# sampotter/butterfly

Measured on AMD Instinct MI355X. Metric: butterfly matvecs/sec (2D Helmholtz HODBF apply), higher is better.
Workload: dtype c128

## Files before the change

butterfly_amd/csrc/bfhip_device.hip:

```cpp

#include <hip/hip_runtime.h>
#include <type_traits>
#include <vector>
#include <stdint.h>
#include <stdio.h>
#include <stdlib.h>

#include "bfhip_internal.h"
#include "bfhip_stage_c128.h"
#include "../../include/bfhip_abi.h"
#include "bfhip_hip.h"
#include "../../include/bfhip_synth.h"

#define BF_WAVES_PER_WG 4
#define BF_WAVE_LDS_BYTES (BF_XCAP * 16)

struct __attribute__((aligned(8))) bfC64 { float re, im; };
struct bfC64Acc { double re, im; };
__device__ __forceinline__ bfC64Acc &operator+=(bfC64Acc &a, bfC64Acc b) { a.re += b.re; a.im += b.im; return a; }

template <int DT> struct Traits;
template <> struct Traits<BFHIP_C128> { using S = double; using A = double; static constexpr int EPL = 1; static constexpr bool CPLX = true; };
template <> struct Traits<BFHIP_F64> { using S = double; using A = double; using E = double; using EA = double; static constexpr int EPL = 2; static constexpr bool CPLX = false; };
template <> struct Traits<BFHIP_F32> { using S = float; using A = float; using E = float; using EA = float; static constexpr int EPL = 4; static constexpr bool CPLX = false; };
template <> struct Traits<BFHIP_C64> { using S = float; using A = double; using E = bfC64; using EA = bfC64Acc; static constexpr int EPL = 2; static constexpr bool CPLX = true; };

__device__ __forceinline__ double bfMac(double acc, double a, double x) { return fma(a, x, acc); }
__device__ __forceinline__ float bfMac(float acc, float a, float x) { return fma(a, x, acc); }
__device__ __forceinline__ bfC64Acc bfMac(bfC64Acc acc, bfC64 a, bfC64 x) {
  double const ar = a.re, ai = a.im, xr = x.re, xi = x.im;
  acc.re = fma(ar, xr, acc.re); acc.re = fma(-ai, xi, acc.re);
  acc.im = fma(ar, xi, acc.im); acc.im = fma(ai, xr, acc.im);
  return acc;
}
__device__ __forceinline__ double bfToAcc(double v) { return v; }
__device__ __forceinline__ float bfToAcc(float v) { return v; }
__device__ __forceinline__ bfC64Acc bfToAcc(bfC64 v) { return bfC64Acc{v.re, v.im}; }
__device__ __forceinline__ double bfFromAcc(double v) { return v; }
__device__ __forceinline__ float bfFromAcc(float v) { return v; }
__device__ __forceinline__ bfC64 bfFromAcc(bfC64Acc v) { return bfC64{(float)v.re, (float)v.im}; }
__device__ __forceinline__ double bfShflXor(double v, int m, int w) { return __shfl_xor(v, m, w); }
__device__ __forceinline__ float bfShflXor(float v, int m, int w) { return __shfl_xor(v, m, w); }
__device__ __forceinline__ bfC64Acc bfShflXor(bfC64Acc v, int m, int w) { return bfC64Acc{__shfl_xor(v.re, m, w), __shfl_xor(v.im, m, w)}; }

template <int NC, typename A, typename S>
__device__ __forceinline__ void bfMacN(A *acc, S const *a, S const *x) {
  if constexpr (NC == 1) {
    acc[0] = fma((A)a[0], (A)x[0], acc[0]);
  } else {
    A const ar = a[0], ai = a[1], xr = x[0], xi = x[1];
    acc[0] = fma(ar, xr, acc[0]); acc[0] = fma(-ai, xi, acc[0]);
    acc[1] = fma(ar, xi, acc[1]); acc[1] = fma(ai, xr, acc[1]);
  }
}

template <typename V> __device__ __forceinline__ V bfLoadStreamV(V const *p) {
  static_assert(sizeof(V) == 16, "one 16-byte lane load");
#if BF_STREAM_NT
  bf_u4 raw = __builtin_nontemporal_load((bf_u4 const *)p);
  V v;
  __builtin_memcpy(&v, &raw, 16);
  return v;
#else
  return *p;
#endif
}

template <bool TL>
__device__ __forceinline__ void bfStageBodyC128(StageParams const &p, double2 (*lds)[BF_XCAP], uint64_t *timeline) {
  int const wave = threadIdx.x >> 6;
  int const lane = threadIdx.x & 63;
  uint32_t const item = __builtin_amdgcn_readfirstlane(blockIdx.x * BF_C128_WG_WAVES + wave);
  if (item >= p.numItems) return;
  BfDevItem const it = p.items[item];
  bfItemC128<TL, false>(p, it, item, lds[wave], lane, timeline, BfNoHook());
}

#ifdef BF_C128_WAVES
#define BF_C128_ATTR __attribute__((amdgpu_waves_per_eu(BF_C128_WAVES, BF_C128_WAVES)))
#else
#define BF_C128_ATTR
#endif
__global__ __launch_bounds__(BF_C128_WG_WAVES * 64) BF_C128_ATTR void bfStageKernelC128(StageParams p) {
  __shared__ __attribute__((aligned(16))) double2 lds[BF_C128_WG_WAVES][BF_XCAP];
  bfStageBodyC128<false>(p, lds, nullptr);
}

#include "bfhip_stage_mfma.h"
#include "bfhip_stage_mfma_blocks.h"

template <int DT, int MR>
__device__ __forceinline__ void bfRowMajorPiece(void const *rowpV, uint32_t upr, typename Traits<DT>::E const *xin, uint32_t n,
                                                uint32_t nrhs, int lane, typename Traits<DT>::EA *racc) {
  using E = typename Traits<DT>::E;
  constexpr int EPL = Traits<DT>::EPL;
  struct __attribute__((aligned(16))) V { E v[EPL]; };
  struct __attribute__((packed, aligned(sizeof(E)))) VU { E v[EPL]; };
  char const *rowp = (char const *)rowpV;
  constexpr int UNR = MR <= 2 ? 4 : 2;
  uint32_t const rowBytes = upr * 16u;
  uint32_t const full = nrhs == 1 ? n / EPL : 0;
  uint32_t u = (uint32_t)lane;
  if (UNR > 1) {
#pragma unroll 1
    for (; u + 64u * (UNR - 1) < full; u += 64u * UNR) {
      V a[UNR][MR];
      VU xv[UNR];
#pragma unroll
      for (int k = 0; k < UNR; ++k) {
#pragma unroll
        for (int r = 0; r < MR; ++r) a[k][r] = bfLoadStreamV((V const *)(rowp + ((uint32_t)r * rowBytes + (u + 64u * k) * 16u)));
      }
#pragma unroll
      for (int k = 0; k < UNR; ++k) xv[k] = *(VU const *)((char const *)xin + (u + 64u * k) * 16u);
#pragma unroll
      for (int k = 0; k < UNR; ++k) {
#pragma unroll
        for (int r = 0; r < MR; ++r) {
#pragma unroll
          for (int e = 0; e < EPL; ++e) racc[r] = bfMac(racc[r], a[k][r].v[e], xv[k].v[e]);
        }
      }
    }
  }
#pragma unroll 1
  for (; u < full; u += 64u) {
    V a[MR];
#pragma unroll
    for (int r = 0; r < MR; ++r) a[r] = bfLoadStreamV((V const *)(rowp + ((uint32_t)r * rowBytes + u * 16u)));
    VU const xv = *(VU const *)((char const *)xin + u * 16u);
#pragma unroll
    for (int r = 0; r < MR; ++r) {
#pragma unroll
      for (int e = 0; e < EPL; ++e) racc[r] = bfMac(racc[r], a[r].v[e], xv.v[e]);
    }
  }
#pragma unroll 1
  for (; u < upr; u += 64u) {
    V a[MR];
#pragma unroll
    for (int r = 0; r < MR; ++r) a[r] = bfLoadStreamV((V const *)(rowp + ((uint32_t)r * rowBytes + u * 16u)));
    E xv[EPL];
#pragma unroll
    for (int e = 0; e < EPL; ++e) xv[e] = u * EPL + e < n ? xin[(uint64_t)(u * EPL + e) * nrhs] : E{};
#pragma unroll
    for (int r = 0; r < MR; ++r) {
#pragma unroll
      for (int e = 0; e < EPL; ++e) racc[r] = bfMac(racc[r], a[r].v[e], xv[e]);
    }
  }
}

template <int DT>
__device__ __forceinline__ void bfStageBodySmall(StageParams const &p, uint32_t const bid) {
  using E = typename Traits<DT>::E;
  using EA = typename Traits<DT>::EA;
  constexpr int EPL = Traits<DT>::EPL;
  constexpr int RMAX = 2 * EPL;
  struct __attribute__((aligned(16))) V { E v[EPL]; };
  int const wave = threadIdx.x >> 6;
  int const lane = threadIdx.x & 63;
  uint32_t const item0 = __builtin_amdgcn_readfirstlane((bid * BF_WAVES_PER_WG + wave) * 4u);
  if (item0 >= p.numItems) return;
  uint32_t const gid = (uint32_t)lane >> 4, gl = (uint32_t)lane & 15u;
  uint32_t const idx = item0 + gid;
  bool const valid = idx < p.numItems;
  BfDevItem it = p.items[valid ? idx : p.numItems - 1];
  uint32_t const mr = valid ? (it.mrFlags & 0xffffu) : 0u;
  uint32_t const np = valid ? it.numPieces : 0u;
  BfDevPiece my;
  my.dataOff = 0; my.inOff = 0; my.ncols = 0; my.flags = 0; my.ld = 0;
  if (gl < np) my = p.pieces[it.pieceBegin + gl];
  uint32_t npMax = 0;
#pragma unroll
  for (int k = 0; k < 4; ++k) {
    uint32_t const v = (uint32_t)__builtin_amdgcn_readlane((int)np, 16 * k);
    npMax = v > npMax ? v : npMax;
  }
  V const *arena = (V const *)p.arena;
  uint32_t const nrhs = p.nrhs;
  E *out = (it.mrFlags & BF_ITEM_OUT_Y) ? (E *)p.y : (E *)p.temp;
  for (uint32_t q = 0; q < nrhs; ++q) {
    EA racc[RMAX];
#pragma unroll
    for (int r = 0; r < RMAX; ++r) racc[r] = EA{};
    EA ident{};
    for (uint32_t k = 0; k < npMax; ++k) {
      int const from = (int)(gid * 16u + k);
      uint32_t const flags = (uint32_t)__shfl((int)my.flags, from, 64);
      uint32_t const inOff = (uint32_t)__shfl((int)my.inOff, from, 64);
      uint32_t const ncols = (uint32_t)__shfl((int)my.ncols, from, 64);
      uint32_t const ld = (uint32_t)__shfl((int)my.ld, from, 64);
      uint32_t const dLo = (uint32_t)__shfl((int)(uint32_t)my.dataOff, from, 64);
      uint32_t const dHi = (uint32_t)__shfl((int)(uint32_t)(my.dataOff >> 32), from, 64);
      if (k >= np) continue;
      E const *xin = ((flags & BF_PIECE_IN_X) ? (E const *)p.x : (E const *)p.temp) + ((uint64_t)inOff * nrhs + q);
      if (flags & BF_PIECE_IDENTITY) {
        if (gl < mr) ident += bfToAcc(xin[(uint64_t)gl * nrhs]);
        continue;
      }
      uint32_t const upr = ld / EPL;
      V const *base = arena + (((uint64_t)dHi << 32) | dLo) / EPL;
#pragma unroll 1
      for (uint32_t u = gl; u < upr; u += 16u) {
        V a[RMAX];
#pragma unroll
        for (int r = 0; r < RMAX; ++r) if ((uint32_t)r < mr) a[r] = bfLoadStreamV(base + (uint64_t)r * upr + u);
        E xv[EPL];
#pragma unroll
        for (int e = 0; e < EPL; ++e) xv[e] = u * EPL + e < ncols ? xin[(uint64_t)(u * EPL + e) * nrhs] : E{};
#pragma unroll
        for (int r = 0; r < RMAX; ++r)
          if ((uint32_t)r < mr) {
#pragma unroll
            for (int e = 0; e < EPL; ++e) racc[r] = bfMac(racc[r], a[r].v[e], xv[e]);
          }
      }
    }
    EA mine = ident;
// ... 128 lines not shown
          if (base && (pc.dataOff != nextOff || base + pc.ncols > BF_MERGE_COLS)) break;
          if (base == 0) data0 = pc.dataOff;
          nextOff = pc.dataOff + (uint64_t)mrPad * pc.ncols;
#pragma unroll
          for (int t = 0; t < XS; ++t) {
            uint32_t const J = (uint32_t)lane + 64u * t - base;
            if (J < pc.ncols) { src[t] = pc.inOff + J; srcX = (pc.flags & BF_PIECE_IN_X) ? srcX | (1u << t) : srcX & ~(1u << t); }
          }
          base += pc.ncols;
        }
        uint32_t n;
        V const *ap = arena + data0 / EPL + lc;
        if (wideCols) {
          E const *xin = (wideFlags & BF_PIECE_IN_X) ? (E const *)p.x : (E const *)p.temp;
          xin += (uint64_t)wideIn * nrhs + q;
          n = wideCols;
          waveSync();
          for (uint32_t j = lane; j < n; j += 64) xs[j] = xin[(uint64_t)j * nrhs];
          waveSync();
        } else if (base) {
          n = base;
          bool const tiny = n <= 2 * g;
          V a2[2];
          if (tiny) {
#pragma unroll
            for (int kk = 0; kk < 2; ++kk) {
#pragma unroll
              for (int e = 0; e < EPL; ++e) a2[kk].v[e] = E{};
              if (active && c + kk * g < n) a2[kk] = bfLoadStreamV(ap + (uint64_t)kk * G);
            }
          }
          E xg[XS];
#pragma unroll
          for (int t = 0; t < XS; ++t)
            xg[t] = src[t] != ~0u ? (((srcX >> t) & 1u) ? (E const *)p.x : (E const *)p.temp)[(uint64_t)src[t] * nrhs + q] : E{};
          waveSync();
#pragma unroll
          for (int t = 0; t < XS; ++t) if ((uint32_t)lane + 64u * t < n) xs[lane + 64 * t] = xg[t];
          waveSync();
          if (tiny) {
#pragma unroll
            for (int kk = 0; kk < 2; ++kk) {
              E xv = (active && c + kk * g < n) ? xs[c + kk * g] : E{};
#pragma unroll
              for (int e = 0; e < EPL; ++e) acc[e] = bfMac(acc[e], a2[kk].v[e], xv);
            }
            continue;
          }
        } else {
          continue;
        }
        uint32_t const nfull = n / g;
        uint32_t j = c;
        uint32_t s = 0;
        V a8[BF_REAL_UNROLL];
#pragma unroll 1
        for (; s + BF_REAL_UNROLL <= nfull; s += BF_REAL_UNROLL) {
#pragma unroll
          for (int k = 0; k < BF_REAL_UNROLL; ++k) a8[k] = bfLoadStreamV(ap + (uint64_t)(s + k) * G);
#pragma unroll
          for (int k = 0; k < BF_REAL_UNROLL; ++k) {
            E const xv = xs[j];
#pragma unroll
            for (int e = 0; e < EPL; ++e) acc[e] = bfMac(acc[e], a8[k].v[e], xv);
            j += g;
          }
        }
        if (s < nfull) {
          uint32_t const left = nfull - s;
#pragma unroll
          for (int k = 0; k < BF_REAL_UNROLL - 1; ++k)
            if ((uint32_t)k < left) a8[k] = bfLoadStreamV(ap + (uint64_t)(s + k) * G);
#pragma unroll
          for (int k = 0; k < BF_REAL_UNROLL - 1; ++k)
            if ((uint32_t)k < left) {
              E const xv = xs[j];
#pragma unroll
              for (int e = 0; e < EPL; ++e) acc[e] = bfMac(acc[e], a8[k].v[e], xv);
              j += g;
            }
        }
        uint32_t const rem = n - nfull * g;
        if (active && c < rem) {
          V a = bfLoadStreamV(ap + (uint64_t)nfull * G);
          E xv = xs[j];
#pragma unroll
          for (int e = 0; e < EPL; ++e) acc[e] = bfMac(acc[e], a.v[e], xv);
        }
      }
    }
    waveSync();
#pragma unroll
    for (int e = 0; e < EPL; ++e) xa[lane * EPL + e] = acc[e];
    waveSync();
    for (uint32_t row = lane; row < mr; row += 64) {
      EA sum{};
      for (uint32_t cc = 0; cc < g; ++cc) sum += xa[cc * mrPad + row];
      out[((uint64_t)it.outOff + row) * nrhs + q] = bfFromAcc(sum);
    }
  }
}

template <int DT>
__global__ __launch_bounds__(BF_WAVES_PER_WG * 64) void bfStageKernelReal(StageParams p) {
  __shared__ __attribute__((aligned(16))) unsigned char ldsRaw[BF_WAVES_PER_WG][BF_WAVE_LDS_BYTES];
  bfStageBodyReal<DT>(p, blockIdx.x, ldsRaw);
}

template <int DT>
__global__ __launch_bounds__(BF_WAVES_PER_WG * 64) __attribute__((amdgpu_waves_per_eu(4, 8))) void bfStageKernelRealBoth(StageParams pr, StageParams ps, uint32_t gridReal) {
  __shared__ __attribute__((aligned(16))) unsigned char ldsRaw[BF_WAVES_PER_WG][BF_WAVE_LDS_BYTES];
  if (blockIdx.x < gridReal) bfStageBodyReal<DT>(pr, blockIdx.x, ldsRaw);
  else bfStageBodySmall<DT>(ps, blockIdx.x - gridReal);
}


#define BF_T_COLS 16
#ifndef BF_T_WIDE_NT
#define BF_T_WIDE_NT 0
#endif
#ifndef BF_T_WIDE_R
#define BF_T_WIDE_R 4
#endif

template <int DT, int R, int NQ, bool COOP, bool ONE, typename CoopBuf>
__device__ __forceinline__ void bfStageBodyT(StageParams const &p, uint32_t const bid, CoopBuf &coopBuf) {
  constexpr int C = 64 / R;
  using S = typename Traits<DT>::S;
  using A = typename Traits<DT>::A;
  constexpr int EPL = Traits<DT>::EPL;
  constexpr int NC = Traits<DT>::CPLX ? 2 : 1;
  constexpr int UNIT = EPL * NC;
  struct __attribute__((aligned(16))) U { S v[UNIT]; };
  int const wave = threadIdx.x >> 6;
  int const lane = threadIdx.x & 63;
  bool const coop = COOP && bid < p.coopItems;
  uint32_t item = __builtin_amdgcn_readfirstlane(coop ? bid : p.coopItems + (bid - p.coopItems) * BF_WAVES_PER_WG + wave);
  if (item >= p.numItems) return;
  uint32_t const wsel = coop ? (uint32_t)wave : 0u, wmask = coop ? BF_WAVES_PER_WG - 1u : 0u;
  BfDevItem const it = p.items[item];
  uint32_t const mr = it.mrFlags & 0xffffu;
  uint32_t const c4 = lane / R, r = lane % R;
  uint32_t jcol[NQ];
#pragma unroll
  for (int cq = 0; cq < NQ; ++cq) jcol[cq] = c4 + C * cq < mr ? c4 + C * cq : mr - 1;
  U const *arena = (U const *)p.arena;
  uint32_t const nrhs = ONE ? 1u : p.nrhs;
  S *out = (it.mrFlags & BF_ITEM_OUT_Y) ? (S *)p.y : (S *)p.temp;
  uint32_t const nq = (mr + C - 1) / C;

  constexpr int CG_RM = (NQ * C) / EPL > 64 ? 64 : (NQ * C) / EPL;
  constexpr int RL_RM = 64 / CG_RM;
  uint32_t const cgRm = lane % CG_RM, rlRm = lane / CG_RM;

  for (uint32_t q = 0; q < nrhs; ++q) {
    A acc[NQ][NC];
#pragma unroll
    for (int cq = 0; cq < NQ; ++cq)
#pragma unroll
      for (int k = 0; k < NC; ++k) acc[cq][k] = 0;
    A racc[EPL][NC];
#pragma unroll
    for (int e = 0; e < EPL; ++e)
#pragma unroll
      for (int k = 0; k < NC; ++k) racc[e][k] = 0;
    bool anyRowMajor = false;
    for (uint32_t wbase = 0; wbase < it.numPieces; wbase += 64) {
      uint32_t const wn = it.numPieces - wbase < 64 ? it.numPieces - wbase : 64;
      BfPieceWin const win = bfPieceWinLoad(p.pieces + it.pieceBegin + wbase, wn, lane);
      uint32_t const pstep = wmask + 1u;
      for (uint32_t pi = wsel; pi < wn; pi += pstep) {
        BfDevPiece const pc = bfPieceWinGet(win, pi);
        S const *xin = (pc.flags & BF_PIECE_IN_X) ? (S const *)p.x : (S const *)p.temp;
        xin += ((uint64_t)pc.inOff * nrhs + q) * NC;
        if (pc.flags & BF_PIECE_IDENTITY) {
          if (r == 0) {
#pragma unroll
            for (int cq = 0; cq < NQ; ++cq)
#pragma unroll
              for (int k = 0; k < NC; ++k) acc[cq][k] += (A)xin[(uint64_t)jcol[cq] * nrhs * NC + k];
          }
          continue;
        }
        if constexpr (EPL > 1) {
          if (pc.flags & BF_PIECE_ROWMAJOR) {
            anyRowMajor = true;
            uint32_t const n = pc.ncols;
            uint32_t const cgc = cgRm < (mr + EPL - 1) / EPL ? cgRm : (mr - 1) / EPL;
            U const *src = arena + pc.dataOff / EPL + cgc;
            uint32_t const rowUnits = pc.ld / EPL;
            constexpr int ITERS = (2 * EPL + RL_RM - 1) / RL_RM;
            bool dual = pi + pstep < wn;
            BfDevPiece pc2 = pc;
            if (dual) {
              pc2 = bfPieceWinGet(win, pi + pstep);
              dual = (pc2.flags & (BF_PIECE_ROWMAJOR | BF_PIECE_IDENTITY)) == BF_PIECE_ROWMAJOR;
            }
            U a[ITERS], a2[ITERS];
            S xv[ITERS][NC], xv2[ITERS][NC];
#pragma unroll
            for (int i = 0; i < ITERS; ++i) {
              uint32_t const srow = rlRm + (uint32_t)i * RL_RM, sc = srow < n ? srow : n - 1;
              a[i] = bfLoadStreamV(src + (uint64_t)sc * rowUnits);
#pragma unroll
              for (int k = 0; k < NC; ++k) {
                S const xr = xin[(uint64_t)sc * nrhs * NC + k];
                xv[i][k] = srow < n ? xr : (S)0;
              }
            }
            if (dual) {
              S const *xin2 = ((pc2.flags & BF_PIECE_IN_X) ? (S const *)p.x : (S const *)p.temp) + ((uint64_t)pc2.inOff * nrhs + q) * NC;
              uint32_t const n2 = pc2.ncols;
              U const *src2 = arena + pc2.dataOff / EPL + cgc;
              uint32_t const rowUnits2 = pc2.ld / EPL;
#pragma unroll
              for (int i = 0; i < ITERS; ++i) {
                uint32_t const srow = rlRm + (uint32_t)i * RL_RM, sc = srow < n2 ? srow : n2 - 1;
                a2[i] = bfLoadStreamV(src2 + (uint64_t)sc * rowUnits2);
#pragma unroll
                for (int k = 0; k < NC; ++k) {
                  S const xr = xin2[(uint64_t)sc * nrhs * NC + k];
                  xv2[i][k] = srow < n2 ? xr : (S)0;
                }
              }
            }
#pragma unroll
            for (int i = 0; i < ITERS; ++i)
#pragma unroll
              for (int e = 0; e < EPL; ++e) bfMacN<NC>(racc[e], &a[i].v[e * NC], xv[i]);
            if (dual) {
#pragma unroll
              for (int i = 0; i < ITERS; ++i)
#pragma unroll
                for (int e = 0; e < EPL; ++e) bfMacN<NC>(racc[e], &a2[i].v[e * NC], xv2[i]);
              pi += pstep;
            }
            continue;
          }
        }
        uint32_t const stride = pc.ld / EPL;
        uint32_t const n = pc.ncols;
        uint32_t const units = (n + EPL - 1) / EPL;
        U const *src = arena + pc.dataOff / EPL;
        for (uint32_t rb = 0; rb < units; rb += R) {
          uint32_t const ru = rb + r < units ? rb + r : units - 1;
          U a[NQ];
#pragma unroll
          for (int cq = 0; cq < NQ; ++cq) if ((uint32_t)cq < nq) a[cq] = (R >= 16 || BF_T_WIDE_NT) ? bfLoadStreamV(src + jcol[cq] * stride + ru) : src[jcol[cq] * stride + ru];
          S xv[UNIT];
#pragma unroll
          for (int e = 0; e < EPL; ++e) {
            uint32_t const row = (rb + r) * EPL + e;
            uint32_t const rowc = row < n ? row : n - 1;
#pragma unroll
            for (int k = 0; k < NC; ++k) {
              S const v = xin[(uint64_t)rowc * nrhs * NC + k];
              xv[e * NC + k] = row < n ? v : (S)0;
            }
          }
#pragma unroll
          for (int cq = 0; cq < NQ; ++cq) {
            if ((uint32_t)cq >= nq) continue;
#pragma unroll
            for (int e = 0; e < EPL; ++e) bfMacN<NC>(acc[cq], &a[cq].v[e * NC], &xv[e * NC]);
          }
        }
      }
    }
#pragma unroll
    for (int m = 1; m < R; m <<= 1)
#pragma unroll
      for (int cq = 0; cq < NQ; ++cq)
#pragma unroll
        for (int k = 0; k < NC; ++k) acc[cq][k] += __shfl_xor(acc[cq][k], m, R);
    if constexpr (EPL > 1) {
      if (anyRowMajor) {
#pragma unroll
        for (int e = 0; e < EPL; ++e)
#pragma unroll
          for (int k = 0; k < NC; ++k)
#pragma unroll
            for (int m = CG_RM; m < 64; m <<= 1) racc[e][k] += __shfl_xor(racc[e][k], m, 64);
#pragma unroll
        for (int cq = 0; cq < NQ; ++cq) {
          uint32_t const col = c4 + C * cq < mr ? c4 + C * cq : 0;
#pragma unroll
          for (int e = 0; e < EPL; ++e)
#pragma unroll
            for (int k = 0; k < NC; ++k) {
              A const t = __shfl(racc[e][k], (int)(col / EPL), 64);
              if ((int)(col % EPL) == e) acc[cq][k] += t;
            }
        }
      }
    }
    if (COOP && coop) {
      if (r == 0) {
#pragma unroll
        for (int cq = 0; cq < NQ; ++cq)
#pragma unroll
          for (int k = 0; k < NC; ++k) coopBuf[wave][c4 + C * cq][k] = acc[cq][k];
      }
      __syncthreads();
      if (wave == 0 && r == 0) {
#pragma unroll
        for (int cq = 0; cq < NQ; ++cq)
#pragma unroll
          for (int k = 0; k < NC; ++k) {
            A t = coopBuf[0][c4 + C * cq][k];
#pragma unroll
            for (int w = 1; w < BF_WAVES_PER_WG; ++w) t += coopBuf[w][c4 + C * cq][k];
            acc[cq][k] = t;
          }
      }
      __syncthreads();
      if (wave != 0) continue;
    }
    if (r == 0) {
#pragma unroll
      for (int cq = 0; cq < NQ; ++cq)
        if (c4 + C * cq < mr)
#pragma unroll
          for (int k = 0; k < NC; ++k) out[(((uint64_t)it.outOff + c4 + C * cq) * nrhs + q) * NC + k] = (S)acc[cq][k];
    }
  }
}

template <int DT, int R, int NQ, bool COOP, bool ONE>
__global__ __launch_bounds__(BF_WAVES_PER_WG * 64) void bfStageKernelT(StageParams p) {
  using A = typename Traits<DT>::A;
  constexpr int NC = Traits<DT>::CPLX ? 2 : 1;
  __shared__ A coopBuf[COOP ? BF_WAVES_PER_WG : 1][COOP ? NQ * (64 / R) : 1][NC];
  bfStageBodyT<DT, R, NQ, COOP, ONE>(p, blockIdx.x, coopBuf);
}

template <int DT, bool ONE>
__global__ __launch_bounds__(BF_WAVES_PER_WG * 64) void bfStageKernelTBoth(StageParams pn, StageParams pw, uint32_t gridNarrow) {
  using A = typename Traits<DT>::A;
  constexpr int NC = Traits<DT>::CPLX ? 2 : 1;
  __shared__ A coopBuf[BF_WAVES_PER_WG][64][NC];
  if (blockIdx.x < gridNarrow) bfStageBodyT<DT, 16, 4, true, ONE>(pn, blockIdx.x, coopBuf);
  else bfStageBodyT<DT, BF_T_WIDE_R, BF_T_WIDE_R, true, ONE>(pw, blockIdx.x - gridNarrow, coopBuf);
}

struct ReduceBatch {
  uint32_t count, nrhs;
  void const *temp;
  struct Entry {
    uint32_t const *rowInterval, *ivBegin;
    int64_t const *srcBias;
    uint64_t numRows;
    void *dest;
    uint32_t blockBegin, pad;
  } e[BF_REDUCE_BATCH];
};

template <typename T, int NC, bool LONG = false>
__global__ __launch_bounds__(256) void bfReduceKernel(ReduceBatch const B) {
  using TA = typename std::conditional<NC == 2 && sizeof(T) == 4, double, T>::type;
  uint32_t k = 0;
  while (k + 1 < B.count && B.e[k + 1].blockBegin <= blockIdx.x) ++k;
  ReduceBatch::Entry const &E = B.e[k];
  uint32_t const nrhs = B.nrhs;
  uint64_t idx = (uint64_t)(blockIdx.x - E.blockBegin) * 256 + threadIdx.x;
  uint64_t total = E.numRows * nrhs;
  if (idx >= total) return;
  uint64_t row = idx / nrhs;
  uint32_t q = (uint32_t)(idx - row * nrhs);
  uint32_t iv = E.rowInterval[row];
  if (iv == 0xffffffffu) return;
  uint32_t b = E.ivBegin[iv], e = E.ivBegin[iv + 1];
  T const *temp = (T const *)B.temp;
  T *dest = (T *)E.dest;
  TA acc[NC];
#pragma unroll
  for (int c = 0; c < NC; ++c) acc[c] = 0;
  uint32_t s = b;
  if (LONG) {
    for (; s + 32 <= e; s += 32) {
      T v[32][NC];
#pragma unroll
      for (int k = 0; k < 32; ++k) {
        T const *src = temp + ((uint64_t)(E.srcBias[s + k] + (int64_t)row) * nrhs + q) * NC;
#pragma unroll
        for (int c = 0; c < NC; ++c) v[k][c] = src[c];
      }
#pragma unroll
      for (int k = 0; k < 32; ++k)
#pragma unroll
        for (int c = 0; c < NC; ++c) acc[c] += v[k][c];
    }
  }
#pragma unroll 8
  for (; s < e; ++s) {
    T const *src = temp + ((uint64_t)(E.srcBias[s] + (int64_t)row) * nrhs + q) * NC;
#pragma unroll
    for (int c = 0; c < NC; ++c) acc[c] += src[c];
  }
#pragma unroll
  for (int c = 0; c < NC; ++c) dest[idx * NC + c] = (T)acc[c];
}

template <typename S>
__global__ __launch_bounds__(256) void bfScalePermuteKernel(S *dst, S const *src, S const *scale, int power, uint64_t const *perm, uint64_t n) {
  uint64_t const i = (uint64_t)blockIdx.x * 256 + threadIdx.x;
  if (i >= n) return;
  S v = src[i];
  if (scale) { S const g = scale[i]; v *= power == 2 ? g * g : g; }
  uint64_t const j = perm ? perm[i] : i;
  if (j < n) dst[j] = v;
}

template <int DT>
__global__ __launch_bounds__(256) void bfSynthKernel(void *arenaV, BfSynthPiece const *pieces, uint64_t seed) {
  using S = typename Traits<DT>::S;
  constexpr bool CPLX = Traits<DT>::CPLX;
  BfSynthPiece const pc = pieces[blockIdx.x];
  uint64_t total = pc.rowMajor ? (uint64_t)pc.mr * pc.ldr : (uint64_t)pc.mrPad * pc.ncols;
  S *dst = (S *)arenaV + pc.dataOff * (CPLX ? 2 : 1);
  for (uint64_t e = threadIdx.x; e < total; e += 256) {
    uint32_t col, r;
    if (pc.rowMajor) { r = (uint32_t)(e / pc.ldr); col = (uint32_t)(e - (uint64_t)r * pc.ldr); }
    else { col = (uint32_t)(e / pc.mrPad); r = (uint32_t)(e - (uint64_t)col * pc.mrPad); }
    S re = 0, im = 0;
    if (r < pc.mr && col < pc.ncols) {
      uint64_t idx = pc.vbase + (uint64_t)(pc.row0 + r) * pc.strideR + (uint64_t)(pc.col0 + col) * pc.strideC;
      re = (S)(bfhip_synth_value(seed, idx, 0) * pc.scale);
      if (CPLX) im = (S)(bfhip_synth_value(seed, idx, 1) * pc.scale);
    }
    if (CPLX) { dst[2 * e] = re; dst[2 * e + 1] = im; }
    else dst[e] = re;
  }
}


#define BF_REAL_CASES(DT, NAME) \
  case BFHIP_KERNEL_REAL_##NAME: hipLaunchKernelGGL(bfStageKernelReal<DT>, dim3(grid), dim3(BF_WAVES_PER_WG * 64), 0, s, p); break; \
  case BFHIP_KERNEL_SMALL_##NAME: hipLaunchKernelGGL(bfStageKernelSmall<DT>, dim3(grid), dim3(BF_WAVES_PER_WG * 64), 0, s, p); break; \
  case BFHIP_KERNEL_REALBOTH_##NAME: hipLaunchKernelGGL(bfStageKernelRealBoth<DT>, dim3(grid + grid2), dim3(BF_WAVES_PER_WG * 64), 0, s, p, p2, grid); break;
#define BF_T_CASES(DT, NAME) \
  case BFHIP_KERNEL_T_##NAME##_NARROW_N: hipLaunchKernelGGL((bfStageKernelT<DT, 16, 4, false, false>), dim3(grid), dim3(BF_WAVES_PER_WG * 64), 0, s, p); break; \
  case BFHIP_KERNEL_T_##NAME##_NARROW_ONE: hipLaunchKernelGGL((bfStageKernelT<DT, 16, 4, false, true>), dim3(grid), dim3(BF_WAVES_PER_WG * 64), 0, s, p); break; \
  case BFHIP_KERNEL_T_##NAME##_NARROW_COOP_N: hipLaunchKernelGGL((bfStageKernelT<DT, 16, 4, true, false>), dim3(grid), dim3(BF_WAVES_PER_WG * 64), 0, s, p); break; \
  case BFHIP_KERNEL_T_##NAME##_NARROW_COOP_ONE: hipLaunchKernelGGL((bfStageKernelT<DT, 16, 4, true, true>), dim3(grid), dim3(BF_WAVES_PER_WG * 64), 0, s, p); break; \
  case BFHIP_KERNEL_T_##NAME##_WIDE_N: hipLaunchKernelGGL((bfStageKernelT<DT, BF_T_WIDE_R, BF_T_WIDE_R, false, false>), dim3(grid), dim3(BF_WAVES_PER_WG * 64), 0, s, p); break; \
  case BFHIP_KERNEL_T_##NAME##_WIDE_ONE: hipLaunchKernelGGL((bfStageKernelT<DT, BF_T_WIDE_R, BF_T_WIDE_R, false, true>), dim3(grid), dim3(BF_WAVES_PER_WG * 64), 0, s, p); break; \
  case BFHIP_KERNEL_T_##NAME##_WIDE_COOP_N: hipLaunchKernelGGL((bfStageKernelT<DT, BF_T_WIDE_R, BF_T_WIDE_R, true, false>), dim3(grid), dim3(BF_WAVES_PER_WG * 64), 0, s, p); break; \
  case BFHIP_KERNEL_T_##NAME##_WIDE_COOP_ONE: hipLaunchKernelGGL((bfStageKernelT<DT, BF_T_WIDE_R, BF_T_WIDE_R, true, true>), dim3(grid), dim3(BF_WAVES_PER_WG * 64), 0, s, p); break;
#define BF_TBOTH_CASES(DT, NAME) \
  case BFHIP_KERNEL_TBOTH_##NAME##_N: hipLaunchKernelGGL((bfStageKernelTBoth<DT, false>), dim3(grid + grid2), dim3(BF_WAVES_PER_WG * 64), 0, s, p, p2, grid); break; \
  case BFHIP_KERNEL_TBOTH_##NAME##_ONE: hipLaunchKernelGGL((bfStageKernelTBoth<DT, true>), dim3(grid + grid2), dim3(BF_WAVES_PER_WG * 64), 0, s, p, p2, grid); break;
static int bfLaunchWaveStage(BfKernelLaunch const &L, BfLaunchArgs const *a, StageParams p, hipStream_t s) {
  bool const small = L.kernel >= BFHIP_KERNEL_SMALL_F64 && L.kernel <= BFHIP_KERNEL_SMALL_C64;
  uint32_t const perWg = small ? 4 * BF_WAVES_PER_WG : BF_WAVES_PER_WG;
  p.items = (BfDevItem const *)a->items + L.first[0];
  p.numItems = (uint32_t)L.count[0];
  p.coopItems = (uint32_t)L.coop[0];
  uint32_t const grid = (uint32_t)(L.coop[0] + (L.count[0] - L.coop[0] + perWg - 1) / perWg);
  StageParams p2 = p;
  uint32_t grid2 = 0;
  if (L.numRanges == 2) {
    bool const tboth = L.kernel >= BFHIP_KERNEL_TBOTH_F64_N && L.kernel <= BFHIP_KERNEL_TBOTH_C64_ONE;
    uint32_t const perWg2 = tboth ? BF_WAVES_PER_WG : 4 * BF_WAVES_PER_WG;
    p2.items = (BfDevItem const *)a->items + L.first[1];
    p2.numItems = (uint32_t)L.count[1];
    p2.coopItems = (uint32_t)L.coop[1];
    grid2 = (uint32_t)(L.coop[1] + (L.count[1] - L.coop[1] + perWg2 - 1) / perWg2);
  }
  switch (L.kernel) {
    BF_REAL_CASES(BFHIP_F64, F64) BF_REAL_CASES(BFHIP_F32, F32) BF_REAL_CASES(BFHIP_C64, C64)
    BF_T_CASES(BFHIP_C128, C128) BF_T_CASES(BFHIP_F64, F64) BF_T_CASES(BFHIP_F32, F32) BF_T_CASES(BFHIP_C64, C64)
    BF_TBOTH_CASES(BFHIP_F64, F64) BF_TBOTH_CASES(BFHIP_F32, F32) BF_TBOTH_CASES(BFHIP_C64, C64)
    default: return bfhipFail(BFABI_ERROR_RUNTIME_ERROR, "internal: kernel id %u is not a wavefront-per-item stage kernel", L.kernel);
  }
  return 0;
}
#undef BF_REAL_CASES
#undef BF_T_CASES
#undef BF_TBOTH_CASES

extern "C" {

// ... 180 lines not shown
```

butterfly_amd/csrc/bfhip_file.c:

```c
#include "bfhip_operator.h"
#include "../../include/bfhip_abi.h"

#include <stdio.h>
#include <stdlib.h>
#include <string.h>

#define BFHIP_FILE_MAGIC "BFHIPOP1"

typedef struct FileHeader {
  char magic[8];
  uint32_t version, dtype, srcDtype, elemSize, epl, xcap, hasTplan, reserved;
  uint64_t numRows, numCols, arenaElems, leafElems, numLeaves, leafBytesAlgorithmic;
} FileHeader;

typedef struct FilePlanHeader { uint64_t numStages, tempElems, numRows, numCols; uint32_t maxItemRows, transposed; } FilePlanHeader;
typedef struct FileStageHeader { uint64_t numItems, numPieces, leafElems, vecIn, vecOut, numReduce; uint32_t maxRows, reserved; } FileStageHeader;
typedef struct FileReduceHeader { uint64_t destOff, numRows, numIntervals, numSrc; uint32_t destSpace, reserved; } FileReduceHeader;

static int writeAll(FILE *fp, void const *p, size_t n) { return n == 0 || fwrite(p, 1, n, fp) == n ? 0 : bfhipFail(BFABI_ERROR_FILE_ERROR, "short write"); }
static int readAll(FILE *fp, void *p, size_t n) { return n == 0 || fread(p, 1, n, fp) == n ? 0 : bfhipFail(BFABI_ERROR_FILE_ERROR, "short read / truncated file"); }

static int writeDeviceArray(FILE *fp, void const *d, size_t bytes) {
  if (!bytes) return 0;
  size_t const chunk = (size_t)64 << 20;
  void *h = malloc(bytes < chunk ? bytes : chunk);
  if (!h) return bfhipFail(BFABI_ERROR_MEMORY_ERROR, "host OOM");
  int rc = 0;
  for (size_t off = 0; off < bytes && !rc; off += chunk) {
    size_t n = bytes - off < chunk ? bytes - off : chunk;
    rc = bfdevMemcpyD2H(h, (char const *)d + off, n);
    if (!rc) rc = writeAll(fp, h, n);
  }
  free(h);
  return rc;
}
static int readDeviceArray(FILE *fp, void **d, size_t bytes, uint64_t *meta) {
  int rc = bfdevMalloc(d, bytes + BF_ARENA_SLACK);
  if (rc || !bytes) return rc;
  if (meta) *meta += bytes;
  size_t const chunk = (size_t)64 << 20;
  void *h = malloc(bytes < chunk ? bytes : chunk);
  if (!h) return bfhipFail(BFABI_ERROR_MEMORY_ERROR, "host OOM");
  for (size_t off = 0; off < bytes && !rc; off += chunk) {
    size_t n = bytes - off < chunk ? bytes - off : chunk;
    rc = readAll(fp, h, n);
    if (!rc) rc = bfdevMemcpyH2D((char *)*d + off, h, n);
  }
  free(h);
  return rc;
}

static int savePlan(FILE *fp, BfPlan const *pl) {
  FilePlanHeader ph = {pl->numStages, pl->tempElems, pl->numRows, pl->numCols, pl->maxItemRows, (uint32_t)pl->transposed};
  int rc = writeAll(fp, &ph, sizeof ph);
  for (uint64_t s = 0; s < pl->numStages && !rc; ++s) {
    BfStage const *st = &pl->stages[s];
    FileStageHeader sh = {st->numItems, st->numPieces, st->leafElems, st->vecIn, st->vecOut, st->numReduce, st->maxRows, 0};
    rc = writeAll(fp, &sh, sizeof sh);
    if (!rc) rc = writeDeviceArray(fp, st->dItems, st->numItems * sizeof(BfDevItem));
    if (!rc) rc = writeDeviceArray(fp, st->dPieces, st->numPieces * sizeof(BfDevPiece));
    for (uint64_t r = 0; r < st->numReduce && !rc; ++r) {
      BfReduce const *rd = &st->reduce[r];
      FileReduceHeader rh = {rd->destOff, rd->numRows, rd->numIntervals, rd->numSrc, rd->destSpace, 0};
      rc = writeAll(fp, &rh, sizeof rh);
      if (!rc) rc = writeDeviceArray(fp, rd->dRowInterval, rd->numRows * 4);
      if (!rc) rc = writeDeviceArray(fp, rd->dIvBegin, (rd->numIntervals + 1) * 4);
      if (!rc) rc = writeDeviceArray(fp, rd->dSrcBias, rd->numSrc * 8);
    }
  }
  return rc;
}

static int readMetaArray(FILE *fp, void **d, void **h, size_t bytes, uint64_t *meta) {
  *h = NULL;
  int rc = bfdevMalloc(d, bytes);
  if (rc || !bytes) return rc;
  if (meta) *meta += bytes;
  *h = malloc(bytes);
  if (!*h) return bfhipFail(BFABI_ERROR_MEMORY_ERROR, "host OOM");
  if ((rc = readAll(fp, *h, bytes))) return rc;
  return bfdevMemcpyH2D(*d, *h, bytes);
}

static int fitsIn(uint64_t off, uint64_t ext, uint64_t len) { return off <= len && ext <= len - off; }
static uint64_t mulAddSat(uint64_t a, uint64_t b, uint64_t c) {
  uint64_t r;
  if (__builtin_mul_overflow(a, b, &r) || __builtin_add_overflow(r, c, &r)) return UINT64_MAX;
  return r;
}

static int validateStage(BfPlan const *pl, uint64_t arenaElems, BfStage const *st, BfDevItem const *items, BfDevPiece const *pieces) {
  uint64_t const inX = pl->numCols, outY = pl->numRows, temp = pl->tempElems;
  for (uint64_t i = 0; i < st->numItems; ++i) {
    BfDevItem const *it = &items[i];
    uint32_t const mr = it->mrFlags & 0xffffu;
    uint64_t const outLen = (it->mrFlags & BF_ITEM_OUT_Y) ? outY : temp;
    if (!mr || mr > pl->maxItemRows || mr > st->maxRows || (it->mrFlags & ~(0xffffu | BF_ITEM_OUT_Y | BF_ITEM_ROWMAJOR | BF_ITEM_MERGED | BF_ITEM_SMALL | BF_ITEM_TNARROW)) ||
        ((it->mrFlags & BF_ITEM_TNARROW) != 0) != (i < st->numNarrow) || ((it->mrFlags & BF_ITEM_TNARROW) && (!pl->transposed || mr > 16)) ||
        ((it->mrFlags & BF_ITEM_SMALL) != 0) != (i >= st->firstSmall) ||
        ((it->mrFlags & BF_ITEM_ROWMAJOR) && (pl->transposed || bfDtypeC128Layout(pl->dtype) || mr > 2 * pl->epl)) ||
        (pl->transposed && mr > 64) ||
        !fitsIn(it->outOff, mr, outLen) || !fitsIn(it->pieceBegin, it->numPieces, st->numPieces))
      return bfhipFail(BFABI_ERROR_FILE_ERROR, "corrupt operator file: item %llu out of bounds", (unsigned long long)i);
    uint32_t const mrPad = (mr + pl->epl - 1) / pl->epl * pl->epl;
    if (it->mrFlags & (BF_ITEM_MERGED | BF_ITEM_SMALL)) {
      int const sm = (it->mrFlags & BF_ITEM_SMALL) != 0;
      uint64_t next = 0, dense = 0;
      int const smRm = sm && (it->mrFlags & BF_ITEM_ROWMAJOR);
      int badm = pl->transposed || bfDtypeC128Layout(pl->dtype) || (!sm && (it->mrFlags & BF_ITEM_ROWMAJOR)) || it->numPieces > (sm ? BF_SMALL_PIECES : 64u) ||
                 (sm && (mr > 2 * pl->epl || !(it->mrFlags & BF_ITEM_ROWMAJOR)));
      for (uint32_t k = 0; k < it->numPieces && !badm; ++k) {
        BfDevPiece const *pc = &pieces[it->pieceBegin + k];
        if (pc->flags & BF_PIECE_IDENTITY) continue;
        if (!smRm && dense && pc->dataOff != next) badm = 1;
        next = mulAddSat(mrPad, pc->ncols, pc->dataOff); dense += pc->ncols;
      }
      if (badm || (!dense && !sm) || dense > (sm ? BF_SMALL_COLS : BF_MERGE_COLS))
        return bfhipFail(BFABI_ERROR_FILE_ERROR, "corrupt operator file: merged item %llu is not one block", (unsigned long long)i);
    }
    for (uint32_t k = 0; k < it->numPieces; ++k) {
      BfDevPiece const *pc = &pieces[it->pieceBegin + k];
      uint64_t const inLen = (pc->flags & BF_PIECE_IN_X) ? inX : temp;
      int bad = (pc->flags & ~(BF_PIECE_IN_X | BF_PIECE_IDENTITY | BF_PIECE_ROWMAJOR)) != 0;
      int const rm = (pc->flags & BF_PIECE_ROWMAJOR) != 0;
      if (!(pc->flags & BF_PIECE_IDENTITY) && !pl->transposed && rm != ((it->mrFlags & BF_ITEM_ROWMAJOR) != 0)) bad = 1;
      if (pc->flags & BF_PIECE_IDENTITY) bad |= !fitsIn(pc->inOff, mr, inLen);
      else if (pl->transposed && rm)
        bad |= !pc->ld || pc->ld % pl->epl || pc->dataOff % pl->epl || bfDtypeC128Layout(pl->dtype) || !pc->ncols ||
               !fitsIn(pc->dataOff, mulAddSat(pc->ncols - 1, pc->ld, (mr + pl->epl - 1) / pl->epl * pl->epl), arenaElems) ||
               !fitsIn(pc->inOff, pc->ncols, inLen);
      else if (rm)
        bad |= !pc->ncols || pc->ld % pl->epl || pc->ld < pc->ncols || pc->dataOff % pl->epl ||
               !fitsIn(pc->dataOff, mulAddSat(mr, pc->ld, 0), arenaElems) || !fitsIn(pc->inOff, pc->ncols, inLen);
      else if (pl->transposed)
        bad |= !pc->ld || pc->ld % pl->epl || pc->ncols > pc->ld || pc->dataOff % pl->epl ||
               !fitsIn(pc->dataOff, mulAddSat(mr - 1, pc->ld, (pc->ncols + pl->epl - 1) / pl->epl * pl->epl), arenaElems) ||
               !fitsIn(pc->inOff, pc->ncols, inLen);
      else
        bad |= !pc->ncols || pc->ncols > pl->xcap || pc->dataOff % pl->epl ||
               !fitsIn(pc->dataOff, mulAddSat(mrPad, pc->ncols, 0), arenaElems) || !fitsIn(pc->inOff, pc->ncols, inLen);
      if (bad) return bfhipFail(BFABI_ERROR_FILE_ERROR, "corrupt operator file: piece %u of item %llu out of bounds", k, (unsigned long long)i);
    }
  }
  return 0;
}

static int validateReduce(BfPlan const *pl, BfReduce const *rd, uint32_t const *rowInterval, uint32_t const *ivBegin, int64_t const *srcBias) {
  uint64_t const destLen = rd->destSpace == BF_SPACE_Y ? pl->numRows : pl->tempElems;
  if ((rd->destSpace != BF_SPACE_Y && rd->destSpace != BF_SPACE_TEMP) || !fitsIn(rd->destOff, rd->numRows, destLen) || rd->numIntervals > rd->numRows + 1)
    return bfhipFail(BFABI_ERROR_FILE_ERROR, "corrupt operator file: reduce destination out of bounds");
  if (ivBegin[0] != 0 || ivBegin[rd->numIntervals] > rd->numSrc) return bfhipFail(BFABI_ERROR_FILE_ERROR, "corrupt operator file: reduce interval table");
  for (uint64_t i = 0; i < rd->numIntervals; ++i)
    if (ivBegin[i + 1] < ivBegin[i]) return bfhipFail(BFABI_ERROR_FILE_ERROR, "corrupt operator file: reduce interval table not monotone");
  for (uint64_t r = 0; r < rd->numRows; ++r) {
    uint32_t const iv = rowInterval[r];
    if (iv == BF_REDUCE_SKIP) continue;
    if (iv >= rd->numIntervals) return bfhipFail(BFABI_ERROR_FILE_ERROR, "corrupt operator file: reduce row %llu", (unsigned long long)r);
    for (uint32_t k = ivBegin[iv]; k < ivBegin[iv + 1]; ++k) {
      int64_t src;
      if (__builtin_add_overflow(srcBias[k], (int64_t)r, &src) || src < 0 || (uint64_t)src >= pl->tempElems) return bfhipFail(BFABI_ERROR_FILE_ERROR, "corrupt operator file: reduce source out of bounds");
    }
  }
  return 0;
}

static int loadPlan(FILE *fp, BfhipOperator *op, BfPlan *pl, FileHeader const *fh, uint64_t arenaElems) {
  FilePlanHeader ph;
  int rc = readAll(fp, &ph, sizeof ph);
  if (rc) return rc;
  if (ph.numStages > (1u << 20) || ph.tempElems >= 0xffffffffu) return bfhipFail(BFABI_ERROR_FILE_ERROR, "corrupt plan header");
  pl->dtype = fh->dtype; pl->elemSize = fh->elemSize; pl->epl = fh->epl; pl->xcap = fh->xcap;
  pl->maxItemRows = ph.maxItemRows; pl->transposed = (int)ph.transposed;
  pl->numRows = ph.numRows; pl->numCols = ph.numCols; pl->numStages = ph.numStages; pl->tempElems = ph.tempElems;
  pl->arenaElems = pl->transposed ? 0 : arenaElems;
  pl->leafElems = fh->leafElems; pl->numLeaves = fh->numLeaves;
  if (pl->epl != 16 / pl->elemSize || pl->xcap != 256 || pl->maxItemRows > 64 * pl->epl || (pl->transposed && pl->maxItemRows > 128))
    return bfhipFail(BFABI_ERROR_FILE_ERROR, "corrupt plan header (lane granule / piece width / item height)");
  pl->stages = calloc(ph.numStages ? ph.numStages : 1, sizeof(BfStage));
  if (!pl->stages) return bfhipFail(BFABI_ERROR_MEMORY_ERROR, "host OOM");
  for (uint64_t s = 0; s < pl->numStages && !rc; ++s) {
    BfStage *st = &pl->stages[s];
    FileStageHeader sh;
    if ((rc = readAll(fp, &sh, sizeof sh))) break;
    if (sh.numItems > 0xffffffffu || sh.numPieces > 0xffffffffu || sh.numReduce > (1u << 20)) { rc = bfhipFail(BFABI_ERROR_FILE_ERROR, "corrupt stage header"); break; }
    st->numItems = sh.numItems; st->numPieces = sh.numPieces; st->leafElems = sh.leafElems; st->vecIn = sh.vecIn; st->vecOut = sh.vecOut;
    st->maxRows = sh.maxRows;
    void *hItems = NULL, *hPieces = NULL;
    rc = readMetaArray(fp, &st->dItems, &hItems, st->numItems * sizeof(BfDevItem), &op->metaBytes);
    if (!rc) rc = readMetaArray(fp, &st->dPieces, &hPieces, st->numPieces * sizeof(BfDevPiece), &op->metaBytes);
    if (!rc) {
      st->firstSmall = st->numItems;
      while (st->firstSmall && (((BfDevItem const *)hItems)[st->firstSmall - 1].mrFlags & BF_ITEM_SMALL)) --st->firstSmall;
      st->numNarrow = 0;
      while (st->numNarrow < st->numItems && (((BfDevItem const *)hItems)[st->numNarrow].mrFlags & BF_ITEM_TNARROW)) ++st->numNarrow;
      rc = validateStage(pl, arenaElems, st, hItems, hPieces);
      if (!rc && pl->transposed) {
        st->maxRowsRest = 0;
        for (uint64_t i = st->numNarrow; i < st->numItems; ++i) {
          uint32_t const mr = ((BfDevItem const *)hItems)[i].mrFlags & 0xffffu;
          if (mr > st->maxRowsRest) st->maxRowsRest = mr;
        }
        st->numCoopNarrow = bfPlanCountCoop(hItems, hPieces, st->numNarrow, pl->elemSize);
        st->numCoop = bfPlanCountCoop((BfDevItem const *)hItems + st->numNarrow, hPieces, st->numItems - st->numNarrow, pl->elemSize);
      }
    }
    free(hItems); free(hPieces);
    if (!rc && sh.numReduce) {
      st->reduce = calloc(sh.numReduce, sizeof(BfReduce));
      if (!st->reduce) rc = bfhipFail(BFABI_ERROR_MEMORY_ERROR, "host OOM");
    }
    for (uint64_t r = 0; r < sh.numReduce && !rc; ++r) {
      BfReduce *rd = &st->reduce[r];
      FileReduceHeader rh;
      if ((rc = readAll(fp, &rh, sizeof rh))) break;
      st->numReduce = r + 1;
      rd->destOff = rh.destOff; rd->numRows = rh.numRows; rd->numIntervals = rh.numIntervals; rd->numSrc = rh.numSrc; rd->destSpace = rh.destSpace;
      if (rd->numRows >= 0xffffffffu || rd->numIntervals >= 0xffffffffu || rd->numSrc >= 0xffffffffu) { rc = bfhipFail(BFABI_ERROR_FILE_ERROR, "corrupt reduce header"); break; }
      void *hRow = NULL, *hIv = NULL, *hBias = NULL;
      rc = readMetaArray(fp, &rd->dRowInterval, &hRow, rd->numRows * 4, &op->metaBytes);
      if (!rc) rc = readMetaArray(fp, &rd->dIvBegin, &hIv, (rd->numIntervals + 1) * 4, &op->metaBytes);
      if (!rc) rc = readMetaArray(fp, &rd->dSrcBias, &hBias, rd->numSrc * 8, &op->metaBytes);
      if (!rc) rc = validateReduce(pl, rd, hRow, hIv, hBias);
      if (!rc) {
        uint32_t const *iv = hIv;
        rd->maxSrc = 0;
        for (uint64_t i = 0; i < rd->numIntervals; ++i) if (iv[i + 1] - iv[i] > rd->maxSrc) rd->maxSrc = iv[i + 1] - iv[i];
      }
      free(hRow); free(hIv); free(hBias);
    }
  }
  return rc;
}

int bfhipSave(BfhipOperator *op, char const *path) {
  if (!op || !path) return bfhipFail(BFABI_ERROR_INVALID_ARGUMENTS, "NULL argument");
  if (op->flags & BFHIP_FLAG_PLAN_ONLY) return bfhipFail(BFABI_ERROR_RUNTIME_ERROR, "a plan-only operator has no device data to save");
  BfDevScope ds;
  int rc = bfDevEnter(&ds, op->device);
  if (rc) return rc;
  if ((rc = bfdevSync(NULL))) goto out;
  FILE *fp = fopen(path, "wb");
  if (!fp) { rc = bfhipFail(BFABI_ERROR_FILE_ERROR, "cannot open %s for writing", path); goto out; }
  FileHeader fh;
  memset(&fh, 0, sizeof fh);
  memcpy(fh.magic, BFHIP_FILE_MAGIC, 8);
  fh.version = 1; fh.dtype = op->plan.dtype; fh.srcDtype = op->srcDtype; fh.elemSize = op->plan.elemSize; fh.epl = op->plan.epl;
  fh.xcap = op->plan.xcap; fh.hasTplan = (uint32_t)op->hasTplan;
  fh.reserved = op->dArenaT ? 1u : 0u;
  fh.numRows = op->plan.numRows; fh.numCols = op->plan.numCols; fh.arenaElems = op->plan.arenaElems;
  fh.leafElems = op->plan.leafElems; fh.numLeaves = op->plan.numLeaves; fh.leafBytesAlgorithmic = op->leafBytesAlgorithmic;
  rc = writeAll(fp, &fh, sizeof fh);
  uint64_t const arenaElemsT = op->dArenaT ? op->tplan.arenaElems : 0;
  if (!rc && op->dArenaT) rc = writeAll(fp, &arenaElemsT, sizeof arenaElemsT);
  if (!rc) rc = savePlan(fp, &op->plan);
  if (!rc && op->hasTplan) rc = savePlan(fp, &op->tplan);
  if (!rc) rc = writeDeviceArray(fp, op->dArena, (size_t)op->plan.arenaElems * op->plan.elemSize);
  if (!rc && op->dArenaT) rc = writeDeviceArray(fp, op->dArenaT, (size_t)arenaElemsT * op->plan.elemSize);
  if (fclose(fp) != 0 && !rc) rc = bfhipFail(BFABI_ERROR_FILE_ERROR, "error closing %s", path);
out:
  bfDevLeave(&ds);
  return rc;
}

int bfhipLoad(char const *path, BfhipOptions const *opts, BfhipOperator **out) {
  if (!path || !out) return bfhipFail(BFABI_ERROR_INVALID_ARGUMENTS, "NULL argument");
  *out = NULL;
  BfhipOptions o;
  memset(&o, 0, sizeof o);
  o.device = -1;
  if (opts) {
    if (opts->structSize < BFHIP_OPTIONS_SIZE_V1) return bfhipFail(BFABI_ERROR_INVALID_ARGUMENTS, "BfhipOptions.structSize too small");
    memcpy(&o, opts, opts->structSize < sizeof o ? opts->structSize : sizeof o);
  }
  if (o.flags & BFHIP_FLAG_PLAN_ONLY) return bfhipFail(BFABI_ERROR_INVALID_ARGUMENTS, "cannot load as plan-only");
  FILE *fp = fopen(path, "rb");
  if (!fp) return bfhipFail(BFABI_ERROR_FILE_ERROR, "cannot open %s", path);
  FileHeader fh;
  int rc = readAll(fp, &fh, sizeof fh);
  if (!rc && (memcmp(fh.magic, BFHIP_FILE_MAGIC, 8) != 0 || fh.version != 1 || fh.dtype > BFHIP_C64 ||
              fh.elemSize != bfDtypeElemSize(fh.dtype) || (fh.dtype == BFHIP_C64 && fh.srcDtype != BFHIP_C128)))
    rc = bfhipFail(BFABI_ERROR_FILE_ERROR, "%s is not a bfhip operator file (bad magic / version / dtype)", path);
  if (rc) { fclose(fp); return rc; }
  BfhipOperator *op = calloc(1, sizeof *op);
  if (!op) { fclose(fp); return bfhipFail(BFABI_ERROR_MEMORY_ERROR, "host OOM"); }
  BfDevScope ds = {0};
  op->flags = o.flags & ~(uint32_t)(BFHIP_FLAG_ADJOINT | BFHIP_FLAG_ADJOINT_PACKED);
  op->srcDtype = fh.srcDtype;
  op->leafBytesAlgorithmic = fh.leafBytesAlgorithmic;
// ... 26 lines not shown
```

Before: 95.55.

## Add software-pipelined load ring for c128 transposed narrow stage kernel

Adds a register ring (default depth 2) for the complex-double transposed stage path with R=16, NQ=4. Loads for the next 16-row chunk of the piece sequence are issued before the current chunk's FMAs, with sched barriers in between, so global-memory latency overlaps compute. The loop is specialized on the number of active column quads, and the kernel gains a waves_per_eu attribute. File validation now rejects leading dimensions of 2^24 or more for this layout, and more live registers could reduce occupancy.

```diff
diff --git a/butterfly_amd/csrc/bfhip_device.hip b/butterfly_amd/csrc/bfhip_device.hip
--- a/butterfly_amd/csrc/bfhip_device.hip
+++ b/butterfly_amd/csrc/bfhip_device.hip
@@ -65,6 +65,8 @@
   return *p;
 #endif
 }
+
+#include "bfhip_stage_t_ring.h"
 
 template <bool TL>
 __device__ __forceinline__ void bfStageBodyC128(StageParams const &p, double2 (*lds)[BF_XCAP], uint64_t *timeline) {
@@ -499,6 +501,7 @@
   constexpr int CG_RM = (NQ * C) / EPL > 64 ? 64 : (NQ * C) / EPL;
   constexpr int RL_RM = 64 / CG_RM;
   uint32_t const cgRm = lane % CG_RM, rlRm = lane / CG_RM;
+  constexpr bool RING = DT == BFHIP_C128 && R == 16 && NQ == 4 && BF_T_RING_DEPTH > 0;
 
   for (uint32_t q = 0; q < nrhs; ++q) {
     A acc[NQ][NC];
@@ -516,7 +519,8 @@
       uint32_t const wn = it.numPieces - wbase < 64 ? it.numPieces - wbase : 64;
       BfPieceWin const win = bfPieceWinLoad(p.pieces + it.pieceBegin + wbase, wn, lane);
       uint32_t const pstep = wmask + 1u;
-      for (uint32_t pi = wsel; pi < wn; pi += pstep) {
+      if constexpr (RING) bfStageTRingC128<BF_T_RING_DEPTH, ONE>(p, win, wn, nrhs, q, wsel, pstep, r, jcol, nq, acc);
+      for (uint32_t pi = wsel; !RING && pi < wn; pi += pstep) {
         BfDevPiece const pc = bfPieceWinGet(win, pi);
         S const *xin = (pc.flags & BF_PIECE_IN_X) ? (S const *)p.x : (S const *)p.temp;
         xin += ((uint64_t)pc.inOff * nrhs + q) * NC;
@@ -674,7 +678,8 @@
 }
 
 template <int DT, int R, int NQ, bool COOP, bool ONE>
-__global__ __launch_bounds__(BF_WAVES_PER_WG * 64) void bfStageKernelT(StageParams p) {
+__global__ __launch_bounds__(BF_WAVES_PER_WG * 64) __attribute__((amdgpu_waves_per_eu(DT == BFHIP_C128 && R == 16 && BF_T_RING_DEPTH > 1 ? BF_T_RING_WAVES : 1, 8)))
+void bfStageKernelT(StageParams p) {
   using A = typename Traits<DT>::A;
   constexpr int NC = Traits<DT>::CPLX ? 2 : 1;
   __shared__ A coopBuf[COOP ? BF_WAVES_PER_WG : 1][COOP ? NQ * (64 / R) : 1][NC];
diff --git a/butterfly_amd/csrc/bfhip_file.c b/butterfly_amd/csrc/bfhip_file.c
--- a/butterfly_amd/csrc/bfhip_file.c
+++ b/butterfly_amd/csrc/bfhip_file.c
@@ -134,6 +134,7 @@
                !fitsIn(pc->dataOff, mulAddSat(mr, pc->ld, 0), arenaElems) || !fitsIn(pc->inOff, pc->ncols, inLen);
       else if (pl->transposed)
         bad |= !pc->ld || pc->ld % pl->epl || pc->ncols > pc->ld || pc->dataOff % pl->epl ||
+               (bfDtypeC128Layout(pl->dtype) && pc->ld >> 24) ||
                !fitsIn(pc->dataOff, mulAddSat(mr - 1, pc->ld, (pc->ncols + pl->epl - 1) / pl->epl * pl->epl), arenaElems) ||
                !fitsIn(pc->inOff, pc->ncols, inLen);
       else
diff --git a/butterfly_amd/csrc/bfhip_stage_t_ring.h b/butterfly_amd/csrc/bfhip_stage_t_ring.h
--- /dev/null
+++ b/butterfly_amd/csrc/bfhip_stage_t_ring.h
@@ -0,0 +1,161 @@
+#ifndef BFHIP_STAGE_T_RING_H
+#define BFHIP_STAGE_T_RING_H
+#include "bfhip_stage_c128.h"
+
+#ifndef BF_T_RING_DEPTH
+#define BF_T_RING_DEPTH 2
+#endif
+#ifndef BF_T_RING_WAVES
+#define BF_T_RING_WAVES 1
+#endif
+
+struct __attribute__((aligned(16))) BfTRingU { double v[2]; };
+struct __attribute__((aligned(8))) BfTRingX { double v[2]; };
+
+template <bool ONE>
+struct BfTRingSeq {
+  StageParams const &p;
+  BfPieceWin const &win;
+  uint32_t const nrhs, q, wn, pstep;
+  uint32_t pi;
+  uint32_t rb, n, stride;
+  char const *leaf, *xin;
+
+  __device__ __forceinline__ BfTRingSeq(StageParams const &p_, BfPieceWin const &win_, uint32_t nrhs_, uint32_t q_, uint32_t wn_, uint32_t wsel, uint32_t pstep_)
+      : p(p_), win(win_), nrhs(nrhs_), q(q_), wn(wn_), pstep(pstep_), pi(wsel) {}
+
+  __device__ __forceinline__ char const *xOf(BfDevPiece const &pc) const {
+    return (char const *)((pc.flags & BF_PIECE_IN_X) ? p.x : (void const *)p.temp) + ((uint64_t)pc.inOff * nrhs + q) * 16u;
+  }
+  __device__ __forceinline__ void decode() {
+    BfDevPiece const pc = bfPieceWinGet(win, pi);
+    xin = xOf(pc);
+    leaf = (char const *)p.arena + pc.dataOff * 16u;
+    n = pc.ncols;
+    stride = pc.ld;
+  }
+  __device__ __forceinline__ void first() { rb = 0; decode(); }
+  __device__ __forceinline__ void next() {
+    bool const adv = rb + 16u >= n;
+    rb = adv ? 0u : rb + 16u;
+    pi = adv ? pi + pstep : pi;
+    decode();
+  }
+};
+
+struct BfTRingSlot {
+  BfTRingU a[4];
+  BfTRingX x;
+  uint32_t nrem;
+};
+
+template <bool ONE>
+__device__ __forceinline__ uint64_t bfTRingXOff(uint32_t e, uint32_t nrhs) {
+  if constexpr (ONE) return e * 16u;
+  else return (uint64_t)e * nrhs * 16u;
+}
+
+template <int NQA, bool ONE>
+__device__ __forceinline__ void bfTRingIssue(BfTRingSlot &s, BfTRingSeq<ONE> const &seq, uint32_t const (&jcol)[4], uint32_t const r) {
+  s.nrem = seq.n - seq.rb;
+  uint32_t const ru = seq.rb + r < seq.n ? seq.rb + r : seq.n - 1u;
+#pragma unroll
+  for (int cq = 0; cq < NQA; ++cq) s.a[cq] = bfLoadStreamV((BfTRingU const *)(seq.leaf + (jcol[cq] * seq.stride + ru) * 16u));
+  s.x = *(BfTRingX const *)(seq.xin + bfTRingXOff<ONE>(ru, seq.nrhs));
+}
+
+template <int NQA>
+__device__ __forceinline__ void bfTRingConsume(BfTRingSlot const &s, double (&acc)[4][2], uint32_t const r) {
+  double xv[2];
+#pragma unroll
+  for (int k = 0; k < 2; ++k) xv[k] = r < s.nrem ? s.x.v[k] : 0.0;
+#pragma unroll
+  for (int cq = 0; cq < NQA; ++cq) bfMacN<2>(acc[cq], s.a[cq].v, xv);
+}
+
+template <int DEPTH, int NQA, bool ONE>
+__device__ __forceinline__ void bfTRingSteps(BfTRingSeq<ONE> &seq, uint32_t const steps, uint32_t const (&jcol)[4], uint32_t const r, double (&acc)[4][2]) {
+  static_assert(DEPTH >= 1 && DEPTH <= 3, "ring written out for 1 - 3 slots");
+  BfTRingSlot s0, s1, s2;
+#define BF_T_ISSUE(S) bfTRingIssue<NQA, ONE>(S, seq, jcol, r)
+#define BF_T_USE(S) bfTRingConsume<NQA>(S, acc, r)
+  seq.first();
+  if (steps < (uint32_t)DEPTH) {
+    BF_T_ISSUE(s0);
+    if (steps == 2) { seq.next(); BF_T_ISSUE(s1); }
+    BF_T_USE(s0);
+    if (steps == 2) BF_T_USE(s1);
+    return;
+  }
+  BF_T_ISSUE(s0); seq.next();
+  if constexpr (DEPTH >= 2) { BF_T_ISSUE(s1); seq.next(); }
+  if constexpr (DEPTH >= 3) { BF_T_ISSUE(s2); seq.next(); }
+  uint32_t left = steps - (uint32_t)DEPTH;
+#pragma unroll 1
+  for (; left >= (uint32_t)DEPTH; left -= (uint32_t)DEPTH) {
+    BF_T_USE(s0); __builtin_amdgcn_sched_barrier(0); BF_T_ISSUE(s0); seq.next(); __builtin_amdgcn_sched_barrier(0);
+    if constexpr (DEPTH >= 2) { BF_T_USE(s1); __builtin_amdgcn_sched_barrier(0); BF_T_ISSUE(s1); seq.next(); __builtin_amdgcn_sched_barrier(0); }
+    if constexpr (DEPTH >= 3) { BF_T_USE(s2); __builtin_amdgcn_sched_barrier(0); BF_T_ISSUE(s2); seq.next(); __builtin_amdgcn_sched_barrier(0); }
+  }
+  if (left == 0) {
+    BF_T_USE(s0);
+    if constexpr (DEPTH >= 2) BF_T_USE(s1);
+    if constexpr (DEPTH >= 3) BF_T_USE(s2);
+  } else if (left == 1) {
+    BF_T_USE(s0); __builtin_amdgcn_sched_barrier(0); BF_T_ISSUE(s0); __builtin_amdgcn_sched_barrier(0);
+    if constexpr (DEPTH >= 2) BF_T_USE(s1);
+    if constexpr (DEPTH >= 3) BF_T_USE(s2);
+    BF_T_USE(s0);
+  } else {
+    BF_T_USE(s0); __builtin_amdgcn_sched_barrier(0); BF_T_ISSUE(s0); seq.next(); __builtin_amdgcn_sched_barrier(0);
+    if constexpr (DEPTH >= 2) { BF_T_USE(s1); __builtin_amdgcn_sched_barrier(0); BF_T_ISSUE(s1); __builtin_amdgcn_sched_barrier(0); }
+    if constexpr (DEPTH >= 3) BF_T_USE(s2);
+    BF_T_USE(s0);
+    if constexpr (DEPTH >= 2) BF_T_USE(s1);
+  }
+#undef BF_T_ISSUE
+#undef BF_T_USE
+}
+
+template <int DEPTH, int NQA, bool ONE>
+__device__ __forceinline__ void bfTRingRun(BfTRingSeq<ONE> &seq, uint32_t const (&jcol)[4], uint32_t const r, double (&acc)[4][2]) {
+  while (seq.pi < seq.wn) {
+    uint32_t steps = 0, pi = seq.pi, fl = 0;
+    bool stop = false;
+    for (; pi < seq.wn; pi += seq.pstep) {
+      fl = (uint32_t)__builtin_amdgcn_readlane((int)seq.win.w[4], (int)pi);
+      uint32_t const n = (uint32_t)__builtin_amdgcn_readlane((int)seq.win.w[3], (int)pi);
+      stop = (fl & BF_PIECE_IDENTITY) || !n;
+      if (stop) break;
+      steps += (n + 15u) >> 4;
+    }
+    if (steps) bfTRingSteps<DEPTH, NQA, ONE>(seq, steps, jcol, r, acc);
+    if (!stop) break;
+    if (fl & BF_PIECE_IDENTITY) {
+      char const *xin = seq.xOf(bfPieceWinGet(seq.win, pi));
+      if (r == 0) {
+#pragma unroll
+        for (int cq = 0; cq < NQA; ++cq) {
+          BfTRingX const v = *(BfTRingX const *)(xin + bfTRingXOff<ONE>(jcol[cq], seq.nrhs));
+#pragma unroll
+          for (int k = 0; k < 2; ++k) acc[cq][k] += v.v[k];
+        }
+      }
+    }
+    seq.pi = pi + seq.pstep;
+  }
+}
+
+template <int DEPTH, bool ONE>
+__device__ __forceinline__ void bfStageTRingC128(StageParams const &p, BfPieceWin const &win, uint32_t wn, uint32_t nrhs, uint32_t q, uint32_t wsel, uint32_t pstep,
+                                                 uint32_t r, uint32_t const (&jcol)[4], uint32_t nq, double (&acc)[4][2]) {
+  BfTRingSeq<ONE> seq(p, win, nrhs, q, wn, (uint32_t)__builtin_amdgcn_readfirstlane((int)wsel), pstep);
+  switch (nq) {
+  case 1: bfTRingRun<DEPTH, 1, ONE>(seq, jcol, r, acc); break;
+  case 2: bfTRingRun<DEPTH, 2, ONE>(seq, jcol, r, acc); break;
+  case 3: bfTRingRun<DEPTH, 3, ONE>(seq, jcol, r, acc); break;
+  default: bfTRingRun<DEPTH, 4, ONE>(seq, jcol, r, acc); break;
+  }
+}
+
+#endif
```

Measured after the change: 95.53. No clear change (-0.0%).
